# YixunLiang/UniTEX

Hardware: AMD Instinct MI355X
Metric: denoising-steps/sec (higher is better)
Workload: dtype bf16

## Files before the change

unitex_amd/_lib.py:

```python
import ctypes as C
import os

_HERE = os.path.dirname(os.path.abspath(__file__))
LIB_PATH = os.path.join(_HERE, "lib", "libunitex_hip.so")

c_void_p, c_long, c_int, c_float = C.c_void_p, C.c_long, C.c_int, C.c_float


class GemmDesc(C.Structure):
    _fields_ = [("A", c_void_p), ("lda", c_long), ("B", c_void_p), ("ldb", c_long),
                ("A2", c_void_p), ("lda2", c_long), ("B2", c_void_p), ("ldb2", c_long),
                ("M", c_int), ("N", c_int), ("K", c_int), ("K2", c_int),
                ("lora_n_limit", c_int), ("lora_seg_n", c_int), ("alpha", c_float),
                ("bias", c_void_p), ("gelu_from", c_int), ("gate", c_void_p),
                ("res", c_void_p), ("ldres", c_long), ("C", c_void_p), ("ldc", c_long),
                ("n_split", c_int), ("C1", c_void_p), ("ldc1", c_long), ("ntn", c_int),
                ("conv_Hi", c_int), ("conv_Wi", c_int), ("conv_Wo", c_int), ("conv_cin_log2", c_int),
                ("conv_stride", c_int), ("conv_pad", c_int), ("conv_up", c_int), ("zero_page", c_void_p),
                ("a_scale", c_void_p), ("lds_a", c_long), ("b_scale", c_void_p), ("lds_b", c_long), ("mx8", c_int),
                ("qk_cols", c_int), ("qk_tok_off", c_int), ("qk_eps", c_float), ("qk_q_scale", c_float),
                ("qk_wq", c_void_p), ("qk_wk", c_void_p), ("qk_cos", c_void_p), ("qk_sin", c_void_p),
                ("qk_Qh", c_void_p), ("qk_Kh", c_void_p), ("qk_hs", c_long),
                ("sk_work", c_void_p), ("sk_work_bytes", C.c_size_t),
                ("q_out", c_void_p), ("ldq_out", c_long), ("qs_out", c_void_p), ("qs_out_rb", c_long), ("q_out_kt0", c_int)]
# ... 177 lines not shown
    "utx_to_u8": (c_int, [c_void_p, c_void_p, c_long, c_long, c_int, c_void_p, c_void_p]),
}

_lib = None


def use_ablation_library():
    global LIB_PATH
    if _lib is not None:
        raise RuntimeError("the library is already loaded")
    LIB_PATH = os.path.join(_HERE, "lib", "libunitex_hip_ablate.so")


def load_library():
    global _lib
    if _lib is not None:
        return _lib
    if not os.path.exists(LIB_PATH):
        raise RuntimeError(
            "libunitex_hip.so not found at %s -- run `python unitex_amd/csrc/build.py` "
            "(or __graft_entry__.build()). There is no CPU/PyTorch fallback by design." % LIB_PATH)
    import torch
    lib = C.CDLL(LIB_PATH)
    for name, (res, args) in SYMBOLS.items():
        fn = getattr(lib, name)
        fn.restype = res
        fn.argtypes = args
    _lib = lib
    return lib


OPTION_NAMES = ["UTX_ATTN_GLDS", "UTX_ATTN_FAST", "UTX_ATTN_Q64", "UTX_ATTN_TPB", "UTX_ATTN_TAILSPLIT",
                "UTX_GEMM_GROUP_M", "UTX_GEMM_TILE", "UTX_GEMM_TAILSPLIT", "UTX_GEMM_PERS_GRID", "UTX_GEMM_PERS_SCHED",
                "UTX_GEMM_STREAMK", "UTX_BVH_STACK_WALK", "UTX_BVH_PACKET", "UTX_ATTN_PEEL", "UTX_ATTN8_PEEL", "UTX_NN_GRID", "UTX_GEMM_FASTK"]


def set_option(name, value):
    rc = load_library().utx_set_option(name.encode(), int(value))
    if rc != 0:
        raise ValueError("utx_set_option(%s) -> %d (%s)" % (name, rc, "ablation-only switch: not in this library" if rc == -7 else "unknown option"))


def get_options():
    lib, out = load_library(), {}
    for n in OPTION_NAMES:
        v = c_int()
        if lib.utx_get_option(n.encode(), C.byref(v)) == 0:
            out[n] = v.value
    return out


def check_abi():
    lib = load_library()
    n = len(ABI_STRUCTS)
    out = (c_int * n)()
    m = lib.utx_abi_sizes(out, n)
    if m != n:
        raise RuntimeError("ABI mismatch: library reports %d descriptor structs, binding has %d" % (m, n))
    for i, st in enumerate(ABI_STRUCTS):
        if C.sizeof(st) != out[i]:
            raise RuntimeError("ABI mismatch for %s: ctypes %d vs C %d" % (st.__name__, C.sizeof(st), out[i]))
    return True


class Context:

    def __init__(self, device=0):
# ... 32 lines not shown
```

unitex_amd/csrc/capi.cpp:

```cpp
#include <cstdint>
#include <hip/hip_runtime.h>
#include <stdio.h>
#include <string.h>
#include <string>
#include <stdlib.h>
#include <mutex>
#include <map>
#include <vector>
#include <utility>
#include "kernels.h"
#include "common.h"

UtxOptions g_utx_opt = {1, 2, 1, 1, 1, 0, 0, 0, 0, 0, 1, 0, 0, 0, 0, 1, 1, 1, 1, 0};

struct OptName { const char* name; int UtxOptions::*field; bool ablation; };
static const OptName kOptions[] = {
    {"UTX_ATTN_GLDS", &UtxOptions::attn_glds, false},       {"UTX_ATTN_FAST", &UtxOptions::attn_fast, false},
    {"UTX_ATTN_Q64", &UtxOptions::attn_q64, false},         {"UTX_ATTN_TPB", &UtxOptions::attn_tpb, false},
    {"UTX_ATTN_TAILSPLIT", &UtxOptions::attn_tailsplit, false},
    {"UTX_GEMM_GROUP_M", &UtxOptions::gemm_group_m, false}, {"UTX_GEMM_TILE", &UtxOptions::gemm_tile, false},
    {"UTX_GEMM_TAILSPLIT", &UtxOptions::gemm_tailsplit, false}, {"UTX_GEMM_PERS_GRID", &UtxOptions::gemm_pers_grid, false},
    {"UTX_GEMM_PERS_SCHED", &UtxOptions::gemm_pers_sched, false}, {"UTX_GEMM_STREAMK", &UtxOptions::gemm_streamk, false},
    {"UTX_BVH_STACK_WALK", &UtxOptions::bvh_stack_walk, false}, {"UTX_BVH_PACKET", &UtxOptions::bvh_packet, false},
    {"UTX_ATTN_PEEL", &UtxOptions::attn_peel, false},             {"UTX_ATTN8_PEEL", &UtxOptions::attn8_peel, false},
    {"UTX_NN_GRID", &UtxOptions::nn_grid, false},                 {"UTX_GEMM_FASTK", &UtxOptions::gemm_fastk, false},
    {"UTX_ATTN_VAR", &UtxOptions::attn_var_abl, true},      {"UTX_ATTN_DEBUG", &UtxOptions::attn_debug_abl, true},
    {"UTX_GEMM_DEBUG", &UtxOptions::gemm_debug_abl, true},
};
#ifdef UTX_ABLATION
static const bool kAblationBuild = true;
#else
static const bool kAblationBuild = false;
#endif

static void options_from_env_once() {
    static std::once_flag once;
    std::call_once(once, [] {
        for (const OptName& o : kOptions) {
            if (o.ablation && !kAblationBuild) continue;
            const char* e = getenv(o.name);
            if (e && *e) g_utx_opt.*(o.field) = atoi(e);
        }
    });
}

struct utx_ctx {
    int device;
    std::string err;
    std::mutex ws_mu;
    std::map<hipStream_t, std::pair<void*, size_t>> attn_ws;
    std::vector<void*> retired;
};

static void* ctx_attn_ws(utx_ctx* ctx, int H, int Sq, int S, hipStream_t stream, size_t* bytes) {
    *bytes = 0;
    if (!ctx) return nullptr;
    const size_t need = utx_attn_workspace_bytes_impl(H, Sq == S ? 0 : Sq, S, utx_ncu());
    if (need == 0) return nullptr;
// ... 429 lines not shown
```

unitex_amd/csrc/gemm_w4.hip:

```cpp
#include "common.h"
#include "kernels.h"
#include "gemm_w4_loop_asm.inc"

#ifndef W4_ZERO_BY_MFMA
#define W4_ZERO_BY_MFMA 1
#endif
#define W4_STAGE 65536

__device__ __forceinline__ float w4_gelu_tanh(float x) {
    const float k0 = 0.7978845608028654f, k1 = 0.044715f;
    const float u = k0 * (x + k1 * x * x * x);
    return x * __builtin_amdgcn_rcpf(1.0f + __expf(-2.0f * u));
}

__device__ __forceinline__ void w4_dma(unsigned lds_addr, unsigned voff, const char* sbase) {
    asm volatile("s_mov_b32 m0, %0\n\ts_nop 0\n\tglobal_load_lds_dwordx4 %1, %2" : : "s"(lds_addr), "v"(voff), "s"(sbase) : "memory");
}
__device__ __forceinline__ void w4_dma_m0(unsigned voff, const char* sbase) {
    asm volatile("global_load_lds_dwordx4 %0, %1" : : "v"(voff), "s"(sbase) : "memory");
}

#define W4_FENCE() __builtin_amdgcn_sched_barrier(0)

__device__ __forceinline__ const char* w4_uniform(const char* p) {
    const unsigned long v = (unsigned long)p;
    const unsigned lo = __builtin_amdgcn_readfirstlane((unsigned)v), hi = __builtin_amdgcn_readfirstlane((unsigned)(v >> 32));
    return (const char*)(((unsigned long)hi << 32) | lo);
}

template <bool GATED, bool QKF = false, bool MX = false, bool FK = false>
__global__ __launch_bounds__(256) __attribute__((amdgpu_waves_per_eu(1, 1))) void gemm256_w4_kernel(GemmParams p, int ntiles, int reserved , int sk_T, int sk_S) {
    extern __shared__ __attribute__((aligned(16))) char smem[];
    const int tid = threadIdx.x;
    const int lane = tid & 63;
    const int wave = __builtin_amdgcn_readfirstlane(tid >> 6);
    const int wm = wave >> 1, wn = wave & 1;
    const int l31 = lane & 31, lh = lane >> 5;
    const int G = gridDim.x;
    const int wid = xcd_remap(blockIdx.x, G);
    const int ntn = p.ntn & 0xffff, group_m = (p.ntn >> 16) & 0xff;
    const int ntm_ = (p.M + 255) / 256;
    const int per_group = group_m * ntn;
    const int nss1 = p.K / 64, nss2 = p.K2 / 64;
    const unsigned ldaB = (unsigned)p.lda * 2, ldbB = (unsigned)p.ldb * 2, lda2B = (unsigned)p.lda2 * 2, ldb2B = (unsigned)p.ldb2 * 2;
    const int nfull_tiles = ntiles - sk_T;
    const int nssu = nss1 + ((p.K2 > 0 && p.lora_n_limit > 0) ? nss2 : 0);
#define W4_NEXT_SEG(tj_, tile_, ok_, k0_, k1_)                                                     \
    do {                                                                                           \
        ok_ = false; k0_ = 0; k1_ = -1;                                                            \
        if (tj_ < 0) {                                                                             \
            tile_ += G;                                                                            \
            if (tile_ < nfull_tiles) ok_ = true; else tj_ = 0;                                     \
        }                                                                                          \
        if (!ok_) {                                                                                \
            const int r_ = wid + tj_ * G;                                                          \
            if (r_ < sk_T * sk_S) {                                                                \
                const int j_ = r_ / sk_T;                                                          \
                ok_ = true; tile_ = nfull_tiles + r_ - j_ * sk_T; ++tj_;                           \
                k0_ = (j_ * nssu) / sk_S; k1_ = ((j_ + 1) * nssu) / sk_S;                          \
            }                                                                                      \
        }                                                                                          \
    } while (0)

#define W4_TILE_ORIGIN(w_, m0_, n0_)                                                       \
// ... 412 lines not shown
                W4_RES_LOAD(rb0, 1, 0); W4_RES_LOAD(rb1, 1, 1); W4_RES_LOAD(rb2, 1, 2); W4_RES_LOAD(rb3, 1, 3);         \
                W4_RES_LOAD(rb4, 1, 4); W4_RES_LOAD(rb5, 1, 5); W4_RES_LOAD(rb6, 1, 6); W4_RES_LOAD(rb7, 1, 7);         \
                W4_FENCE();                                                                                            \
                W4_GATE_BLOCK(0, ra, 15, 1, true)                                                                      \
                W4_GATE_BLOCK(1, rb, 23, 1, true)                                                                      \
                W4_GATE_BLOCK(2, ra, 30, -1, false)                                                                    \
                W4_GATE_BLOCK(3, rb, 22, -1, false)                                                                    \
            } else {                                                                                                   \
                W4_GATE_SLOW_BLOCK(0) W4_GATE_SLOW_BLOCK(1) W4_GATE_SLOW_BLOCK(2) W4_GATE_SLOW_BLOCK(3)                \
            }                                                                                                          \
        } else if (QKF && c_n0 < p.qk_cols) {                                                                         \
                                             \
            const int col0 = c_n0 + wn * 128, dq = p.qk_cols >> 1;                                                      \
            const bool isk = col0 >= dq;                                                                               \
            const int head = (isk ? col0 - dq : col0) >> 7;                                                            \
            const float qs = isk ? 1.0f : p.qk_q_scale;                                                                \
            const int qsrow0 = p.qk_tok_off + c_m0 + wm * 128, qsrow_max = p.qk_tok_off + p.M - 1;                      \
            const unsigned qvo = (unsigned)((elane >> 4) * 256 + (elane & 15) * 16);                                    \
            const char* const qdst = (const char*)(isk ? p.qk_Kh : p.qk_Qh);                                          \
            const unsigned qhead = (unsigned)head * (unsigned)p.qk_hs * 2u;         \
            W4_QK_BLOCK(0) W4_QK_BLOCK(1) W4_QK_BLOCK(2) W4_QK_BLOCK(3)                                                \
        } else if (MX && !GATED && do_gelu && p.q_out) {                                                              \
                     \
            const int qc0 = c_n0 + wn * 128 - p.gelu_from;                                                             \
            uint8_t* const mxq_b = (uint8_t*)p.q_out + (long)(c_m0 + wm * 128) * p.ldq_out + qc0;                      \
            const unsigned mxq_vo = (unsigned)((elane >> 4) * (unsigned)p.ldq_out + (unsigned)(elane & 15) * 8u);      \
            uint32_t* const mxq_s = (uint32_t*)p.qs_out + ((long)(p.q_out_kt0 + (qc0 >> 7)) * p.qs_out_rb + ((c_m0 >> 7) + wm)) * 128; \
            W4_MXQ_BLOCK(0) W4_MXQ_BLOCK(1) W4_MXQ_BLOCK(2) W4_MXQ_BLOCK(3)                                            \
        } else {                                                                                                       \
            if (do_gelu) { W4_PLAIN_BLOCK(0, true) W4_PLAIN_BLOCK(1, true) W4_PLAIN_BLOCK(2, true) W4_PLAIN_BLOCK(3, true) } \
            else { W4_PLAIN_BLOCK(0, false) W4_PLAIN_BLOCK(1, false) W4_PLAIN_BLOCK(2, false) W4_PLAIN_BLOCK(3, false) } \
        }                                                                                                              \
    } while (0)

#define W4_DUMP(slot_)                                                                                                 \
    do {                                                                                                               \
        int dlane = lane;                                                                                              \
        asm volatile("" : "+v"(dlane));                                                                                \
        float* const wsb = (float*)p.sk_work + ((long)(slot_) * 4 + wave) * 16384 + dlane * 4;                         \
        _Pragma("unroll") for (int jn_ = 0; jn_ < 4; ++jn_)                                                            \
        _Pragma("unroll") for (int im_ = 0; im_ < 4; ++im_)                                                            \
        _Pragma("unroll") for (int a_ = 0; a_ < 4; ++a_) {                                                             \
            const w4_f32x4 v_ = {W4_ACC(jn_, im_, 4 * a_), W4_ACC(jn_, im_, 4 * a_ + 1), W4_ACC(jn_, im_, 4 * a_ + 2), W4_ACC(jn_, im_, 4 * a_ + 3)}; \
            *reinterpret_cast<w4_f32x4*>(wsb + ((jn_ * 4 + im_) * 4 + a_) * 256) = v_;                                 \
        }                                                                                                              \
    } while (0)

#define W4_STAGE_HALF(isb_) do { W4_DMA(isb_, 0); W4_DMA(isb_, 1); W4_DMA(isb_, 2); W4_DMA(isb_, 3); W4_DMA(isb_, 4); W4_DMA(isb_, 5); W4_DMA(isb_, 6); W4_DMA(isb_, 7); } while (0)
    W4_STAGE_AT(0, -1, false);
#define W4_XREAD16(FA_, FB_, base_, xlo_, xhi_)                                                            \
    W4_XREAD(0, FA_, FB_, base_, xlo_, xhi_); W4_XREAD(1, FA_, FB_, base_, xlo_, xhi_); W4_XREAD(2, FA_, FB_, base_, xlo_, xhi_); W4_XREAD(3, FA_, FB_, base_, xlo_, xhi_);     \
    W4_XREAD(4, FA_, FB_, base_, xlo_, xhi_); W4_XREAD(5, FA_, FB_, base_, xlo_, xhi_); W4_XREAD(6, FA_, FB_, base_, xlo_, xhi_); W4_XREAD(7, FA_, FB_, base_, xlo_, xhi_);     \
    W4_XREAD(8, FA_, FB_, base_, xlo_, xhi_); W4_XREAD(9, FA_, FB_, base_, xlo_, xhi_); W4_XREAD(10, FA_, FB_, base_, xlo_, xhi_); W4_XREAD(11, FA_, FB_, base_, xlo_, xhi_);   \
    W4_XREAD(12, FA_, FB_, base_, xlo_, xhi_); W4_XREAD(13, FA_, FB_, base_, xlo_, xhi_); W4_XREAD(14, FA_, FB_, base_, xlo_, xhi_); W4_XREAD(15, FA_, FB_, base_, xlo_, xhi_);
    if constexpr (MX) {
        W4_STAGE_HALF(0); W4_STAGE_HALF(1);
        W4_XSCALE_LOAD(sa_nxt, s_pSA); W4_XSCALE_LOAD(sb_nxt, s_pSB);
        W4_STAGE_ADVANCE();
        W4_DMA(0, 0); W4_DMA(0, 1); W4_DMA(0, 2); W4_DMA(0, 3); W4_DMA(0, 4); W4_DMA(0, 5); W4_DMA(0, 6); W4_DMA(0, 7);
        W4_DMA(1, 0); W4_DMA(1, 1); W4_DMA(1, 2);
        W4_WAIT_VM(11);
        W4_LANDED2(sa_nxt, sb_nxt);
        W4_FENCE();
        W4_XSCALE_TAKE();
        W4_COMPUTE_AT(0, -1);
        __builtin_amdgcn_s_barrier();
// ... 4 lines not shown
    } else {
    W4_STAGE_HALF(0); W4_STAGE_HALF(1); W4_STAGE_ADVANCE();
    W4_DMA(0, 0); W4_DMA(0, 1); W4_DMA(0, 2); W4_DMA(0, 3); W4_DMA(0, 4); W4_DMA(0, 5);
    asm volatile("s_waitcnt vmcnt(6)" ::: "memory");
    W4_COMPUTE_AT(0, -1);
    __builtin_amdgcn_s_barrier();
    W4_FENCE();
#pragma unroll
    for (int r = 0; r < 8; ++r) W4_READ(r, fa0, fb0, 0, xk0);
    asm volatile("s_waitcnt lgkmcnt(0)" ::: "memory");
    W4_FENCE();
    }

    unsigned w4f_ra[2][4], w4f_rb[2][4];
    if constexpr (FK && !MX) {
        const int xk_[4] = {xk0, xk1, xk2, xk3};
#pragma unroll
        for (int sl = 0; sl < 2; ++sl)
#pragma unroll
            for (int k = 0; k < 4; ++k) { w4f_ra[sl][k] = lds0 + (unsigned)(sl * W4_STAGE + arow + xk_[k]); w4f_rb[sl][k] = lds0 + (unsigned)(sl * W4_STAGE + brow + xk_[k]); }
    }
    for (;;) {
        if constexpr (FK && !MX) {
            if (c_slot == 0) {
                int n_ = (s_seg_end - s_ss - 1) >> 1;
                const int nc_ = (c_nss - c_ss - 1) >> 1;
                if (nc_ < n_) n_ = nc_;
                if (n_ > 0) {
                    const unsigned long pa_ = (unsigned long)s_pA, pb_ = (unsigned long)s_pB;
                    const unsigned w4f_pa_lo = __builtin_amdgcn_readfirstlane((unsigned)pa_), w4f_pa_hi = __builtin_amdgcn_readfirstlane((unsigned)(pa_ >> 32));
                    const unsigned w4f_pb_lo = __builtin_amdgcn_readfirstlane((unsigned)pb_), w4f_pb_hi = __builtin_amdgcn_readfirstlane((unsigned)(pb_ >> 32));
                    const unsigned w4f_trips = __builtin_amdgcn_readfirstlane((unsigned)n_);
                    const unsigned w4f_ldsdma = __builtin_amdgcn_readfirstlane(lds0 + (unsigned)wave * 1024u);
                    asm volatile(W4F_ASM_TEXT : W4F_ASM_OUTPUTS : W4F_ASM_INPUTS : W4F_ASM_CLOBBERS);
                    s_pA += 256L * n_; s_pB += 256L * n_;
                    s_ss += 2 * n_; c_ss += 2 * n_;
                }
            }
        }
        const int cb = c_slot * W4_STAGE, nb = (c_slot ^ 1) * W4_STAGE;
#define W4_PIECE_OF(ks_, i_) ((ks_) == 3 ? (((i_) % 3) == 0 ? (i_) / 3 : -1) : (ks_) == 0 ? (((i_) % 3) == 2 ? 6 + (i_) / 3 : -1) \
                              : (ks_) == 1 ? ((((i_) % 3) == 1 && (i_) < 15) ? 11 + (i_) / 3 : -1) : -1)
#define W4_KSTEP(i_, ks_, FA_, FB_, FAn_, FBn_, base_, xk_)                                                \
        {                                                                                                  \
            constexpr int pc_ = W4_PIECE_OF(ks_, i_);                                                      \
            constexpr int isb_ = pc_ >= 8 ? 1 : 0, d_ = pc_ < 0 ? 0 : (pc_ & 7);                           \
            if constexpr (pc_ >= 0) W4_MF_M0(i_, FA_, FB_, W4_DMA_LDS(isb_, d_)); else W4_MF(i_, FA_, FB_); \
            W4_FENCE();                                                                                    \
            if ((i_) < 8) W4_READ(i_, FAn_, FBn_, base_, xk_);                                             \
            if constexpr (pc_ >= 0) W4_DMA_M0(isb_, d_);                                                   \
            W4_FENCE();                                                                                    \
        }
#define W4_KSTEP16(ks_, FA_, FB_, FAn_, FBn_, base_, xk_)                                                  \
        W4_KSTEP(0, ks_, FA_, FB_, FAn_, FBn_, base_, xk_) W4_KSTEP(1, ks_, FA_, FB_, FAn_, FBn_, base_, xk_)   \
        W4_KSTEP(2, ks_, FA_, FB_, FAn_, FBn_, base_, xk_) W4_KSTEP(3, ks_, FA_, FB_, FAn_, FBn_, base_, xk_)   \
        W4_KSTEP(4, ks_, FA_, FB_, FAn_, FBn_, base_, xk_) W4_KSTEP(5, ks_, FA_, FB_, FAn_, FBn_, base_, xk_)   \
        W4_KSTEP(6, ks_, FA_, FB_, FAn_, FBn_, base_, xk_) W4_KSTEP(7, ks_, FA_, FB_, FAn_, FBn_, base_, xk_)   \
        W4_KSTEP(8, ks_, FA_, FB_, FAn_, FBn_, base_, xk_) W4_KSTEP(9, ks_, FA_, FB_, FAn_, FBn_, base_, xk_)   \
        W4_KSTEP(10, ks_, FA_, FB_, FAn_, FBn_, base_, xk_) W4_KSTEP(11, ks_, FA_, FB_, FAn_, FBn_, base_, xk_) \
        W4_KSTEP(12, ks_, FA_, FB_, FAn_, FBn_, base_, xk_) W4_KSTEP(13, ks_, FA_, FB_, FAn_, FBn_, base_, xk_) \
        W4_KSTEP(14, ks_, FA_, FB_, FAn_, FBn_, base_, xk_) W4_KSTEP(15, ks_, FA_, FB_, FAn_, FBn_, base_, xk_)
#define W4_XPIECE_OF(ks_, i_) ((ks_) == 1 ? ((((i_) % 3) != 2) ? ((i_) / 3) * 2 + ((i_) % 3) : -1) : (((((i_) % 3) != 2) && (i_) < 7) ? 11 + ((i_) / 3) * 2 + ((i_) % 3) : -1))
#define W4_XKSTEP(i_, ks_, FA_, FB_, FAn_, FBn_, base_, xlo_, xhi_)                                        \
        {                                                                                                  \
            constexpr int pc_ = W4_XPIECE_OF(ks_, i_);                                                     \
            constexpr int isb_ = pc_ >= 8 ? 1 : 0, d_ = pc_ < 0 ? 0 : (pc_ & 7);                           \
            if constexpr (pc_ >= 0) W4_XMF_M0(i_, ks_, FA_, FB_, xlds + (unsigned)(isb_ * 32768 + d_ * 4096)); else W4_XMF(i_, ks_, FA_, FB_); \
            W4_FENCE();                                                                                    \
            W4_XREAD(i_, FAn_, FBn_, base_, xlo_, xhi_);                                                   \
            if constexpr (pc_ >= 0) W4_DMA_M0(isb_, d_);                                                   \
            if constexpr ((ks_) == 0 && (i_) == 0) W4_XSCALE_LOAD(sa_nxt, s_pSA);                          \
            if constexpr ((ks_) == 0 && (i_) == 1) W4_XSCALE_LOAD(sb_nxt, s_pSB);                          \
            W4_FENCE();                                                                                    \
        }
#define W4_XKSTEP16(ks_, FA_, FB_, FAn_, FBn_, base_, xlo_, xhi_)                                          \
        W4_XKSTEP(0, ks_, FA_, FB_, FAn_, FBn_, base_, xlo_, xhi_) W4_XKSTEP(1, ks_, FA_, FB_, FAn_, FBn_, base_, xlo_, xhi_)   \
        W4_XKSTEP(2, ks_, FA_, FB_, FAn_, FBn_, base_, xlo_, xhi_) W4_XKSTEP(3, ks_, FA_, FB_, FAn_, FBn_, base_, xlo_, xhi_)   \
        W4_XKSTEP(4, ks_, FA_, FB_, FAn_, FBn_, base_, xlo_, xhi_) W4_XKSTEP(5, ks_, FA_, FB_, FAn_, FBn_, base_, xlo_, xhi_)   \
        W4_XKSTEP(6, ks_, FA_, FB_, FAn_, FBn_, base_, xlo_, xhi_) W4_XKSTEP(7, ks_, FA_, FB_, FAn_, FBn_, base_, xlo_, xhi_)   \
        W4_XKSTEP(8, ks_, FA_, FB_, FAn_, FBn_, base_, xlo_, xhi_) W4_XKSTEP(9, ks_, FA_, FB_, FAn_, FBn_, base_, xlo_, xhi_)   \
        W4_XKSTEP(10, ks_, FA_, FB_, FAn_, FBn_, base_, xlo_, xhi_) W4_XKSTEP(11, ks_, FA_, FB_, FAn_, FBn_, base_, xlo_, xhi_) \
        W4_XKSTEP(12, ks_, FA_, FB_, FAn_, FBn_, base_, xlo_, xhi_) W4_XKSTEP(13, ks_, FA_, FB_, FAn_, FBn_, base_, xlo_, xhi_) \
        W4_XKSTEP(14, ks_, FA_, FB_, FAn_, FBn_, base_, xlo_, xhi_) W4_XKSTEP(15, ks_, FA_, FB_, FAn_, FBn_, base_, xlo_, xhi_)
        if constexpr (MX) {
            unsigned xlds = lds_w + (unsigned)s_slot * W4_STAGE;
            W4_XKSTEP16(0, xa0, xb0, xa1, xb1, cb, xk2, xk3)
            W4_STAGE_ADVANCE();
            xlds = lds_w + (unsigned)s_slot * W4_STAGE;
            asm volatile("s_waitcnt lgkmcnt(0)" ::: "memory");
            W4_WAIT_VM(0);
            W4_LANDED2(sa_nxt, sb_nxt);
            W4_FENCE();
            __builtin_amdgcn_s_barrier();
            W4_FENCE();
            W4_XKSTEP16(1, xa1, xb1, xa0, xb0, nb, xk0, xk1)
            asm volatile("s_waitcnt lgkmcnt(0)" ::: "memory");
            W4_FENCE();
            W4_XSCALE_TAKE();
            W4_FENCE();
        } else {
        W4_KSTEP16(0, fa0, fb0, fa1, fb1, cb, xk1)
        asm volatile("s_waitcnt lgkmcnt(0)" ::: "memory");
        W4_FENCE();
        W4_KSTEP16(1, fa1, fb1, fa0, fb0, cb, xk2)
        W4_STAGE_ADVANCE();
        asm volatile("s_waitcnt lgkmcnt(0)" ::: "memory");
        W4_FENCE();
        W4_KSTEP16(2, fa0, fb0, fa1, fb1, cb, xk3)
        asm volatile("s_waitcnt lgkmcnt(0)" ::: "memory");
        asm volatile("s_waitcnt vmcnt(0)" ::: "memory");
        W4_FENCE();
        __builtin_amdgcn_s_barrier();
        W4_FENCE();
        W4_KSTEP16(3, fa1, fb1, fa0, fb0, nb, xk0)
        asm volatile("s_waitcnt lgkmcnt(0)" ::: "memory");
        W4_FENCE();
        }
        c_slot ^= 1;
        ++c_ss;
        if (c_ss != c_nss) continue;
        const bool full = (c_m0 + 256 <= p.M);
        W4_MFMA_DRAIN();
        if (c_tj > 0) { W4_DUMP(wid + (c_tj - 1) * G); }
        else W4_EPILOGUE();
        W4_ZERO_ACC()
        if constexpr (MX) {
            const int rb = c_slot * W4_STAGE;
            W4_XREAD16(xa0, xb0, rb, xk0, xk1)
            asm volatile("s_waitcnt lgkmcnt(0)" ::: "memory");
            W4_FENCE();
        }
        if constexpr (QKF) {
            const int rb = c_slot * W4_STAGE;
#pragma unroll
            for (int r = 0; r < 8; ++r) W4_READ(r, fa0, fb0, rb, xk0);
            asm volatile("s_waitcnt lgkmcnt(0)" ::: "memory");
            W4_FENCE();
        }
        bool done;
        W4_COMPUTE_NEXT(done);
        if (done) break;
    }
    asm volatile("s_waitcnt vmcnt(0)" ::: "memory");
}

template <bool GATED>
__global__ __launch_bounds__(256) void gemm_w4_fixup_kernel(GemmParams p, int ntiles, int sk_T, int sk_S) {
    typedef __attribute__((ext_vector_type(4))) float f32x4v;
    const int t = blockIdx.x >> 4, wv = (blockIdx.x >> 2) & 3, im = blockIdx.x & 3;
    const int tid = threadIdx.x, lane = tid & 63, jn = tid >> 6, l31 = lane & 31, lh = lane >> 5;
    const int wm = wv >> 1, wn = wv & 1;
    const int ntn = p.ntn & 0xffff, group_m = (p.ntn >> 16) & 0xff, ntm = (p.M + 255) / 256, per_group = group_m * ntn;
    const int w = ntiles - sk_T + t;
    const int grp = w / per_group, rem = w - grp * per_group, ftm = grp * group_m;
    const int gs = (ntm - ftm < group_m) ? ntm - ftm : group_m;
    const int tn = rem / gs;
    const int m0 = (ftm + rem - tn * gs) * 256, n0 = tn * 256;
    f32x4v acc[4];
#pragma unroll
    for (int a = 0; a < 4; ++a) acc[a] = f32x4v{0.f, 0.f, 0.f, 0.f};
    for (int j = 0; j < sk_S; ++j) {
        const float* src = (const float*)p.sk_work + ((long)(j * sk_T + t) * 4 + wv) * 16384 + (jn * 4 + im) * 1024 + lane * 4;
#pragma unroll
        for (int a = 0; a < 4; ++a) acc[a] += *reinterpret_cast<const f32x4v*>(src + a * 256);
    }
    const int m = m0 + wm * 128 + im * 32 + l31;
    if (m >= p.M) return;
    const bool do_gelu = !GATED && n0 >= p.gelu_from, to_c1 = !GATED && n0 >= p.n_split;
    bf16_t* const crow = to_c1 ? (bf16_t*)p.C1 + (long)m * p.ldc1 - p.n_split : (bf16_t*)p.C + (long)m * p.ldc;
#pragma unroll
    for (int a = 0; a < 4; ++a) {
        const int n = n0 + wn * 128 + jn * 32 + 8 * a + 4 * lh;
        float v[4];
// ... 39 lines not shown
    const int nssu = p.K / 64 + ((p.K2 > 0 && p.lora_n_limit > 0) ? p.K2 / 64 : 0);
    if (opt >= 1000) {
        const int S = opt - 1000;
        if (S >= 2 && S <= 8 && nssu >= S && T * S <= 2 * grid) { *T_out = T; *S_out = S; }
        return;
    }
    const int margin = opt > 1 ? opt : 4;
    int best = nssu - margin, bestS = 0;
    for (int S = 2; S <= 8; ++S) {
        if (nssu / S < 8 || T * S > 2 * grid) break;
        const int passes = (T * S + grid - 1) / grid;
        const int est = passes * ((nssu + S - 1) / S + 4) + 6 + (8 * T * S) / 256;
        if (est < best) { best = est; bestS = S; }
    }
    if (bestS) { *T_out = T; *S_out = bestS; }
}

extern "C" int utx_launch_gemm_w4(GemmParams p, hipStream_t stream) {
    constexpr int LDS = 2 * W4_STAGE + 4 * 8192;
    UTX_ONCE_PER_DEVICE(attr_set) {
        const void* ks[2] = {reinterpret_cast<const void*>(gemm256_w4_kernel<false>), reinterpret_cast<const void*>(gemm256_w4_kernel<true>)};
        for (const void* k : ks)
            if (hipFuncSetAttribute(k, hipFuncAttributeMaxDynamicSharedMemorySize, LDS) != hipSuccess) return -3;
        UTX_ONCE_DONE(attr_set);
    }
    const int ncu = utx_ncu();
    const int ntm = (p.M + 255) / 256, ntn = p.N / 256;
    int group_m = g_utx_opt.gemm_group_m > 0 ? g_utx_opt.gemm_group_m : (ntn >= 32 ? 8 : 2);
    if (group_m > ntm) group_m = ntm;
    p.ntn = ntn | (group_m << 16);
    const int tiles = ntm * ntn;
    int grid = tiles < ncu ? tiles : ncu;
    if (g_utx_opt.gemm_pers_grid > 0 && g_utx_opt.gemm_pers_grid < grid) grid = g_utx_opt.gemm_pers_grid;
    int sk_T = 0, sk_S = 0;
    utx_gemm_w4_split_plan(&p, tiles, grid, (p.sk_work && p.sk_work_bytes >= (size_t)2 * grid * 262144) ? 1 : 0, &sk_T, &sk_S);
    if (p.mx8 == 2) {
        if (p.K2 > 0 || p.qk_cols > 0 || (p.K % 64) || !p.a_scale || !p.b_scale || p.lds_a < (p.M + 127) / 128 || p.lds_b < p.N / 128 ||
            ((uintptr_t)p.a_scale & 15) || ((uintptr_t)p.b_scale & 15)) return -2;
        if (p.gate && (p.gelu_from < p.N || p.n_split < p.N)) return -2;
        if (p.q_out && (p.gate || !p.qs_out || p.gelu_from >= p.N || (p.gelu_from % 128) || (p.ldq_out & 7) || p.ldq_out < p.N - p.gelu_from ||
                        p.qs_out_rb < (p.M + 127) / 128 || p.q_out_kt0 < 0 || ((uintptr_t)p.qs_out & 15) || ((uintptr_t)p.q_out & 7))) return -2;
        UTX_ONCE_PER_DEVICE(ax) {
            if (hipFuncSetAttribute(reinterpret_cast<const void*>(gemm256_w4_kernel<false, false, true>), hipFuncAttributeMaxDynamicSharedMemorySize, LDS) != hipSuccess ||
                hipFuncSetAttribute(reinterpret_cast<const void*>(gemm256_w4_kernel<true, false, true>), hipFuncAttributeMaxDynamicSharedMemorySize, LDS) != hipSuccess) return -3;
            UTX_ONCE_DONE(ax);
        }
        if (p.gate) hipLaunchKernelGGL((gemm256_w4_kernel<true, false, true>), dim3(grid), dim3(256), LDS, stream, p, tiles, 0, sk_T, sk_S);
        else hipLaunchKernelGGL((gemm256_w4_kernel<false, false, true>), dim3(grid), dim3(256), LDS, stream, p, tiles, 0, sk_T, sk_S);
    } else if (g_utx_opt.gemm_fastk != 0) {
        UTX_ONCE_PER_DEVICE(af) {
            const void* kf[3] = {reinterpret_cast<const void*>(gemm256_w4_kernel<false, false, false, true>), reinterpret_cast<const void*>(gemm256_w4_kernel<true, false, false, true>),
                                 reinterpret_cast<const void*>(gemm256_w4_kernel<false, true, false, true>)};
            for (const void* k : kf)
                if (hipFuncSetAttribute(k, hipFuncAttributeMaxDynamicSharedMemorySize, LDS) != hipSuccess) return -3;
            UTX_ONCE_DONE(af);
        }
        if (p.gate) {
            if (p.gelu_from < p.N || p.n_split < p.N) return -2;
            hipLaunchKernelGGL((gemm256_w4_kernel<true, false, false, true>), dim3(grid), dim3(256), LDS, stream, p, tiles, 0, sk_T, sk_S);
        } else if (p.qk_cols > 0) hipLaunchKernelGGL((gemm256_w4_kernel<false, true, false, true>), dim3(grid), dim3(256), LDS, stream, p, tiles, 0, sk_T, sk_S);
        else hipLaunchKernelGGL((gemm256_w4_kernel<false, false, false, true>), dim3(grid), dim3(256), LDS, stream, p, tiles, 0, sk_T, sk_S);
    } else if (p.gate) {
        if (p.gelu_from < p.N || p.n_split < p.N) return -2;
        hipLaunchKernelGGL((gemm256_w4_kernel<true>), dim3(grid), dim3(256), LDS, stream, p, tiles, 0, sk_T, sk_S);
    } else {
        if (p.qk_cols > 0) {
            UTX_ONCE_PER_DEVICE(aq) { if (hipFuncSetAttribute(reinterpret_cast<const void*>(gemm256_w4_kernel<false, true>), hipFuncAttributeMaxDynamicSharedMemorySize, LDS) != hipSuccess) return -3; UTX_ONCE_DONE(aq); }
            hipLaunchKernelGGL((gemm256_w4_kernel<false, true>), dim3(grid), dim3(256), LDS, stream, p, tiles, 0, sk_T, sk_S);
        } else
        hipLaunchKernelGGL((gemm256_w4_kernel<false>), dim3(grid), dim3(256), LDS, stream, p, tiles, 0, sk_T, sk_S);
    }
    if (sk_T > 0) {
        if (p.gate) hipLaunchKernelGGL((gemm_w4_fixup_kernel<true>), dim3(sk_T * 16), dim3(256), 0, stream, p, tiles, sk_T, sk_S);
        else hipLaunchKernelGGL((gemm_w4_fixup_kernel<false>), dim3(sk_T * 16), dim3(256), 0, stream, p, tiles, sk_T, sk_S);
    }
    return hipGetLastError() == hipSuccess ? 0 : -4;
}
```

unitex_amd/csrc/kernels.h:

```cpp
#pragma once
#include <hip/hip_runtime.h>
#include <stdint.h>
#include "../../include/unitex_hip.h"
#ifndef UTX_BF16_T
#define UTX_BF16_T
typedef uint16_t bf16_t;
#endif

struct AttnParams {
    const bf16_t* q;
    const bf16_t* k;
    const bf16_t* vt;
    bf16_t* o;
    long q_hs, q_ss, k_hs, k_ss, vt_hs, vt_ds, o_ss;
    int H, S, nqb;
    int Sq;
    int dbg;
    float scale_log2;
    unsigned char* flags;
    int flag_hs;
    int w_base, nsplit, tiles_per_split;
    bf16_t* part_o;
    float* part_lse;
    float key_bias_log2;
// ... 7 lines not shown
    const uint8_t *q8, *k8;
    const uint8_t* v8t;
    const uint32_t *qs, *ks;
    const uint32_t* vs;
    bf16_t* o;
    long o_ss;
    int H, S, Sq, S_pad, nqb;
    float key_bias_log2;
    int key_bias_period;
    int w_base, nsplit, tiles_per_split;
    bf16_t* part_o;
    float* part_lse;
    void* work;
    size_t work_bytes;
};
struct UtxOptions {
    int attn_glds;
    int attn_fast;
    int attn_q64;
    int attn_tpb;
    int attn_tailsplit;
    int gemm_group_m;
    int gemm_tile;
    int gemm_tailsplit;
    int gemm_pers_grid;
    int gemm_pers_sched;
    int gemm_streamk;
    int bvh_stack_walk;
    int attn_var_abl, attn_debug_abl, gemm_debug_abl;
    int bvh_packet;
    int attn_peel;
    int attn8_peel;
    int gemm_fastk;
    int nn_grid;
};
extern UtxOptions g_utx_opt;

typedef utx_gemm_desc GemmParams;
typedef utx_knn_desc KnnParams;
typedef utx_gemv_desc GemvParams;
typedef utx_qkv_post_desc QkvPostParams;
typedef utx_ln_mod_desc LnModParams;
typedef utx_sched_desc SchedParams;

extern "C" {
int utx_launch_attn_fwd(const void* q, const void* k, const void* vt, void* o,
                        long q_hs, long q_ss, long k_hs, long k_ss, long vt_hs, long vt_ds,
                        long o_ss, int H, int S, int Sq, float scale, float key_bias_log2, int key_bias_period, void* work, size_t work_bytes, hipStream_t stream);
void utx_attn_split_plan_impl(int H, int Sq, int S, int ncu, int out[4]);
size_t utx_attn_workspace_bytes_impl(int H, int Sq, int S, int ncu);
size_t utx_attn_split_bytes_impl(int H, int Sq, int S, int ncu);
size_t utx_attn_q64_flag_bytes(int H, int Sq, int S);
int utx_attn_q64_takes(const AttnParams* p, int presc);
int utx_launch_attn_merge(const AttnParams* t, int n_items, hipStream_t stream);
int utx_launch_attn_fwd_glds(const AttnParams* p, int presc, hipStream_t stream);
int utx_launch_attn_fwd_fp8(const Attn8Params* p, hipStream_t stream);
int utx_launch_quant_vt_mx8(const void* vt, void* v8, void* vs, int H, int S_pad, hipStream_t stream);
int utx_launch_attn_fwd_blk(const void* q, const void* k, const void* vt, void* o, long q_hs, long q_ss, long k_hs, long k_ss, long vt_hs, long vt_ds,
                            long o_ss, int H, int S, int Sq, float scale, float key_bias_log2, int key_bias_period, void* work, size_t work_bytes,
                            int blk_rows, long q_bs, long k_bs, long vt_bs, hipStream_t stream);
int utx_launch_attn_fwd_q64(const AttnParams* p, int presc, hipStream_t stream);
int utx_launch_gemm_bf16(const GemmParams* p, hipStream_t stream);
size_t utx_gemm_streamk_workspace_bytes_impl(void);
void utx_gemm_plan_impl(const GemmParams* p, int ncu, int sk_has_work, int out[4]);
void utx_gemm_w4_split_plan(const GemmParams* p, int tiles, int grid, int has_work, int* T, int* S);
int utx_launch_gemm_w4(GemmParams p, hipStream_t stream);
// ... 48 lines not shown
```

Measured before the change: 0.5705.

## Park GEMM epilogue outputs in registers and drain stores during next tile's K-loop

Adds a 'park' epilogue path to the persistent W4 GEMM kernel for non-gated, non-QK, non-MX variants. Accumulators for the last three row-blocks are scaled, biased, GELU'd and packed to bf16 in registers instead of being written immediately. Their LDS staging and nontemporal global stores are then interleaved into the first K-tiles of the next output tile through per-kstep hooks. If there is no next tile, or the next tile is short, they are flushed directly. This aims to hide epilogue store latency behind MFMA work, at the cost of many extra live VGPRs and more complex scheduling. It is enabled by default through a new UTX_GEMM_PARK option.

Result: slower. 0.5499 (-3.6%).

```diff
diff --git a/unitex_amd/_lib.py b/unitex_amd/_lib.py
--- a/unitex_amd/_lib.py
+++ b/unitex_amd/_lib.py
@@ -233,7 +233,7 @@
 
 OPTION_NAMES = ["UTX_ATTN_GLDS", "UTX_ATTN_FAST", "UTX_ATTN_Q64", "UTX_ATTN_TPB", "UTX_ATTN_TAILSPLIT",
                 "UTX_GEMM_GROUP_M", "UTX_GEMM_TILE", "UTX_GEMM_TAILSPLIT", "UTX_GEMM_PERS_GRID", "UTX_GEMM_PERS_SCHED",
-                "UTX_GEMM_STREAMK", "UTX_BVH_STACK_WALK", "UTX_BVH_PACKET", "UTX_ATTN_PEEL", "UTX_ATTN8_PEEL", "UTX_NN_GRID", "UTX_GEMM_FASTK"]
+                "UTX_GEMM_STREAMK", "UTX_BVH_STACK_WALK", "UTX_BVH_PACKET", "UTX_ATTN_PEEL", "UTX_ATTN8_PEEL", "UTX_NN_GRID", "UTX_GEMM_FASTK", "UTX_GEMM_PARK"]
 
 
 def set_option(name, value):
diff --git a/unitex_amd/csrc/capi.cpp b/unitex_amd/csrc/capi.cpp
--- a/unitex_amd/csrc/capi.cpp
+++ b/unitex_amd/csrc/capi.cpp
@@ -11,7 +11,7 @@
 #include "kernels.h"
 #include "common.h"
 
-UtxOptions g_utx_opt = {1, 2, 1, 1, 1, 0, 0, 0, 0, 0, 1, 0, 0, 0, 0, 1, 1, 1, 1, 0};
+UtxOptions g_utx_opt = {1, 2, 1, 1, 1, 0, 0, 0, 0, 0, 1, 0, 0, 0, 0, 1, 1, 1, 1, 1, 0};
 
 struct OptName { const char* name; int UtxOptions::*field; bool ablation; };
 static const OptName kOptions[] = {
@@ -24,6 +24,7 @@
     {"UTX_BVH_STACK_WALK", &UtxOptions::bvh_stack_walk, false}, {"UTX_BVH_PACKET", &UtxOptions::bvh_packet, false},
     {"UTX_ATTN_PEEL", &UtxOptions::attn_peel, false},             {"UTX_ATTN8_PEEL", &UtxOptions::attn8_peel, false},
     {"UTX_NN_GRID", &UtxOptions::nn_grid, false},                 {"UTX_GEMM_FASTK", &UtxOptions::gemm_fastk, false},
+    {"UTX_GEMM_PARK", &UtxOptions::gemm_park, false},
     {"UTX_ATTN_VAR", &UtxOptions::attn_var_abl, true},      {"UTX_ATTN_DEBUG", &UtxOptions::attn_debug_abl, true},
     {"UTX_GEMM_DEBUG", &UtxOptions::gemm_debug_abl, true},
 };
diff --git a/unitex_amd/csrc/gemm_w4.hip b/unitex_amd/csrc/gemm_w4.hip
--- a/unitex_amd/csrc/gemm_w4.hip
+++ b/unitex_amd/csrc/gemm_w4.hip
@@ -29,7 +29,7 @@
 }
 
 template <bool GATED, bool QKF = false, bool MX = false, bool FK = false>
-__global__ __launch_bounds__(256) __attribute__((amdgpu_waves_per_eu(1, 1))) void gemm256_w4_kernel(GemmParams p, int ntiles, int reserved , int sk_T, int sk_S) {
+__global__ __launch_bounds__(256) __attribute__((amdgpu_waves_per_eu(1, 1))) void gemm256_w4_kernel(GemmParams p, int ntiles, int park , int sk_T, int sk_S) {
     extern __shared__ __attribute__((aligned(16))) char smem[];
     const int tid = threadIdx.x;
     const int lane = tid & 63;
@@ -508,6 +508,97 @@
             else { W4_PLAIN_BLOCK(0, false) W4_PLAIN_BLOCK(1, false) W4_PLAIN_BLOCK(2, false) W4_PLAIN_BLOCK(3, false) } \
         }                                                                                                              \
     } while (0)
+
+#ifndef W4_PARK_FIRST
+#define W4_PARK_FIRST 1
+#endif
+    constexpr bool PARKABLE = !GATED && !QKF && !MX;
+#define W4_PARK_BLOCK(im_, GELU_)                                                                                      \
+        _Pragma("unroll") for (int jn_ = 0; jn_ < 4; ++jn_)                                                            \
+            _Pragma("unroll") for (int q_ = 0; q_ < 2; ++q_) {                                                         \
+                float b8_[8];                                                                                          \
+                _Pragma("unroll") for (int h_ = 0; h_ < 2; ++h_)                                                       \
+                    _Pragma("unroll") for (int d_ = 0; d_ < 2; ++d_) {                                                 \
+                        const uint32_t w_ = bsel[jn_][q_][2 * h_ + d_];                                                \
+                        b8_[4 * h_ + 2 * d_] = p.bias ? bf2f((uint16_t)(w_ & 0xffff)) : 0.f;                           \
+                        b8_[4 * h_ + 2 * d_ + 1] = p.bias ? bf2f((uint16_t)(w_ >> 16)) : 0.f;                          \
+                    }                                                                                                  \
+                float v_[8];                                                                                           \
+                _Pragma("unroll") for (int c_ = 0; c_ < 8; ++c_) {                                                     \
+                    v_[c_] = W4_ACC(jn_, im_, 8 * q_ + c_) * p.alpha + b8_[c_];                                        \
+                    if (GELU_) v_[c_] = w4_gelu_tanh(rbf(v_[c_]));                                                     \
+                }                                                                                                      \
+                pk[im_][jn_][q_][0] = pack2bf(v_[0], v_[1]); pk[im_][jn_][q_][1] = pack2bf(v_[2], v_[3]);              \
+                pk[im_][jn_][q_][2] = pack2bf(v_[4], v_[5]); pk[im_][jn_][q_][3] = pack2bf(v_[6], v_[7]);              \
+                W4_FENCE();       \
+            }
+#define W4_PARK_TILE()                                                                                                 \
+    do {                                                                                                               \
+        int el31 = l31, elh = lh, elane = lane;                                                                        \
+        asm volatile("" : "+v"(el31), "+v"(elh), "+v"(elane));                                                         \
+        const uint32_t hm = 0u - (uint32_t)elh;                                                                        \
+        const bool do_gelu = c_n0 >= p.gelu_from;                                                                      \
+        const bool to_c1 = c_n0 >= p.n_split;                                                                          \
+        bf16_t* const cbase = to_c1 ? (bf16_t*)p.C1 : (bf16_t*)p.C;                                                    \
+        pk_ldc = to_c1 ? p.ldc1 : p.ldc;                                                                               \
+        pk_wofs = el31 * 256; pk_wxor = ((el31 & 15) ^ elh) << 4;                                                      \
+        pk_rofs = (elane >> 4) * 256 + (((elane & 15) ^ (elane >> 4)) << 4);                                           \
+        pk_rowg = c_m0 + wm * 128 + (elane >> 4);                                                                      \
+        pk_rows = p.M - (c_m0 + wm * 128);              \
+        pk_cub = (char*)cbase + ((long)(c_m0 + wm * 128) * pk_ldc + (c_n0 + wn * 128 - (to_c1 ? p.n_split : 0))) * 2;  \
+        pk_cvo = (unsigned)((elane >> 4) * (unsigned)pk_ldc * 2u + (unsigned)(elane & 15) * 16u);                      \
+        const int wofs = pk_wofs, wxor = pk_wxor;                                                                      \
+        const bf16_t* const ebias = (const bf16_t*)(p.bias ? p.bias : p.B) + c_n0 + wn * 128;                          \
+        w4_u32x16 bq0, bq1, bq2, bq3;                                                                                  \
+        uint32_t bsel[4][2][4];                                                                                        \
+        W4_SLOAD64(bq0, bq1, bq2, bq3, ebias);                                                                         \
+        _Pragma("unroll") for (int jn_ = 0; jn_ < 4; ++jn_) {                                                          \
+            const w4_u32x16 bw_ = jn_ == 0 ? bq0 : jn_ == 1 ? bq1 : jn_ == 2 ? bq2 : bq3;                              \
+            _Pragma("unroll") for (int q_ = 0; q_ < 2; ++q_)                                                           \
+                _Pragma("unroll") for (int e_ = 0; e_ < 4; ++e_)                                                       \
+                    bsel[jn_][q_][e_] = (bw_[8 * q_ + 4 * (e_ >> 1) + 2 + (e_ & 1)] & hm) | (bw_[8 * q_ + 4 * (e_ >> 1) + (e_ & 1)] & ~hm); \
+        }                                                                                                              \
+        const long ldc = pk_ldc; char* const cub = pk_cub; const unsigned cvo = pk_cvo; const int rofs = pk_rofs, rowg = pk_rowg;       \
+        if (do_gelu) { W4_PARK_BLOCKS(true) } else { W4_PARK_BLOCKS(false) }                                           \
+    } while (0)
+#define W4_PARK_ONE(im_, GELU_)                                                                                        \
+        if constexpr ((im_) < W4_PARK_FIRST) { W4_PLAIN_BLOCK(im_, GELU_) }                                            \
+        else if constexpr ((im_) == W4_PARK_FIRST) { W4_EPI_WRITE(im_, GELU_) }                                        \
+        else { W4_PARK_BLOCK(im_, GELU_) }
+#define W4_PARK_BLOCKS(GELU_) W4_PARK_ONE(0, GELU_) W4_PARK_ONE(1, GELU_) W4_PARK_ONE(2, GELU_) W4_PARK_ONE(3, GELU_)
+#define W4_PK_STAGE(im_, jn_, q_)                                                                                      \
+        {                                                                                                              \
+            auto s0_ = __builtin_amdgcn_permlane32_swap(pk[im_][jn_][q_][0], pk[im_][jn_][q_][2], false, false);       \
+            auto s1_ = __builtin_amdgcn_permlane32_swap(pk[im_][jn_][q_][1], pk[im_][jn_][q_][3], false, false);       \
+            *reinterpret_cast<uint4*>(stg + pk_wofs + (((4 * (jn_) + 2 * (q_)) << 4) ^ pk_wxor)) = make_uint4(s0_[0], s1_[0], s0_[1], s1_[1]); \
+        }
+#define W4_PK_READ(t_) pky[t_] = *reinterpret_cast<const uint4*>(stg + (t_) * 1024 + (pk_rofs ^ (64 * ((t_) & 3))));
+#define W4_PK_STORE(im_, t_)                                                                                           \
+        if (32 * (im_) + 32 <= pk_rows || pk_rowg + 32 * (im_) + 4 * (t_) < p.M) {                                     \
+            const w4_u32x4 ov_ = {pky[t_].x, pky[t_].y, pky[t_].z, pky[t_].w};                                         \
+            __builtin_nontemporal_store(ov_, reinterpret_cast<w4_u32x4*>(pk_cub + (long)(32 * (im_) + 4 * (t_)) * pk_ldc * 2 + pk_cvo)); \
+        }
+#define W4_DRAIN_SLOT(d_, ks_, i_)                                                                                     \
+        {                                                                                                              \
+            constexpr int s_ = 16 * (ks_) + (i_);                                                                      \
+            if constexpr (s_ >= 4 && s_ <= 18 && (s_ & 1) == 0) { W4_PK_STORE(d_, ((s_ - 4) >> 1) & 7) }               \
+            if constexpr (s_ <= 14 && (s_ & 1) == 0) { W4_PK_READ((s_ >> 1) & 7) }                                     \
+            if constexpr ((d_) < 3 && (ks_) == 2 && (i_) < 8) W4_PK_STAGE(((d_) + 1) & 3, ((i_) & 7) >> 1, (i_) & 1)   \
+        }
+#define W4_DRAIN0(ks_, i_) W4_DRAIN_SLOT(W4_PARK_FIRST, ks_, i_)
+#define W4_DRAIN1(ks_, i_) W4_DRAIN_SLOT(W4_PARK_FIRST + 1, ks_, i_)
+#define W4_DRAIN2(ks_, i_) W4_DRAIN_SLOT(W4_PARK_FIRST + 2, ks_, i_)
+#define W4_DRAIN3(ks_, i_) W4_DRAIN_SLOT(W4_PARK_FIRST + 3, ks_, i_)
+#define W4_PK_FLUSH(im_, staged_)                                                                                      \
+        {                                                                                                              \
+            if (!(staged_)) {                                                                                          \
+                W4_PK_STAGE(im_, 0, 0) W4_PK_STAGE(im_, 0, 1) W4_PK_STAGE(im_, 1, 0) W4_PK_STAGE(im_, 1, 1)            \
+                W4_PK_STAGE(im_, 2, 0) W4_PK_STAGE(im_, 2, 1) W4_PK_STAGE(im_, 3, 0) W4_PK_STAGE(im_, 3, 1)            \
+            }                                                                                                          \
+            W4_PK_READ(0) W4_PK_READ(1) W4_PK_READ(2) W4_PK_READ(3) W4_PK_READ(4) W4_PK_READ(5) W4_PK_READ(6) W4_PK_READ(7) \
+            W4_PK_STORE(im_, 0) W4_PK_STORE(im_, 1) W4_PK_STORE(im_, 2) W4_PK_STORE(im_, 3)                            \
+            W4_PK_STORE(im_, 4) W4_PK_STORE(im_, 5) W4_PK_STORE(im_, 6) W4_PK_STORE(im_, 7)                            \
+        }
 
 #define W4_DUMP(slot_)                                                                                                 \
     do {                                                                                                               \
@@ -578,6 +669,13 @@
                     const unsigned w4f_pb_lo = __builtin_amdgcn_readfirstlane((unsigned)pb_), w4f_pb_hi = __builtin_amdgcn_readfirstlane((unsigned)(pb_ >> 32));
                     const unsigned w4f_trips = __builtin_amdgcn_readfirstlane((unsigned)n_);
                     const unsigned w4f_ldsdma = __builtin_amdgcn_readfirstlane(lds0 + (unsigned)wave * 1024u);
+                    if constexpr (PARKABLE) {
+                        int ar_ = arow, br_ = brow;
+                        asm volatile("" : "+v"(ar_), "+v"(br_));
+                        const int xk_[4] = {xk0, xk1, xk2, xk3};
+                        _Pragma("unroll") for (int sl = 0; sl < 2; ++sl)
+                            _Pragma("unroll") for (int k = 0; k < 4; ++k) { w4f_ra[sl][k] = lds0 + (unsigned)(sl * W4_STAGE + ar_ + xk_[k]); w4f_rb[sl][k] = lds0 + (unsigned)(sl * W4_STAGE + br_ + xk_[k]); }
+                    }
                     asm volatile(W4F_ASM_TEXT : W4F_ASM_OUTPUTS : W4F_ASM_INPUTS : W4F_ASM_CLOBBERS);
                     s_pA += 256L * n_; s_pB += 256L * n_;
                     s_ss += 2 * n_; c_ss += 2 * n_;
@@ -587,7 +685,7 @@
         const int cb = c_slot * W4_STAGE, nb = (c_slot ^ 1) * W4_STAGE;
 #define W4_PIECE_OF(ks_, i_) ((ks_) == 3 ? (((i_) % 3) == 0 ? (i_) / 3 : -1) : (ks_) == 0 ? (((i_) % 3) == 2 ? 6 + (i_) / 3 : -1) \
                               : (ks_) == 1 ? ((((i_) % 3) == 1 && (i_) < 15) ? 11 + (i_) / 3 : -1) : -1)
-#define W4_KSTEP(i_, ks_, FA_, FB_, FAn_, FBn_, base_, xk_)                                                \
+#define W4_KSTEP(i_, ks_, FA_, FB_, FAn_, FBn_, base_, xk_, HOOK_)                                         \
         {                                                                                                  \
             constexpr int pc_ = W4_PIECE_OF(ks_, i_);                                                      \
             constexpr int isb_ = pc_ >= 8 ? 1 : 0, d_ = pc_ < 0 ? 0 : (pc_ & 7);                           \
@@ -595,17 +693,40 @@
             W4_FENCE();                                                                                    \
             if ((i_) < 8) W4_READ(i_, FAn_, FBn_, base_, xk_);                                             \
             if constexpr (pc_ >= 0) W4_DMA_M0(isb_, d_);                                                   \
+            HOOK_(ks_, i_)                                                                                 \
             W4_FENCE();                                                                                    \
         }
-#define W4_KSTEP16(ks_, FA_, FB_, FAn_, FBn_, base_, xk_)                                                  \
-        W4_KSTEP(0, ks_, FA_, FB_, FAn_, FBn_, base_, xk_) W4_KSTEP(1, ks_, FA_, FB_, FAn_, FBn_, base_, xk_)   \
-        W4_KSTEP(2, ks_, FA_, FB_, FAn_, FBn_, base_, xk_) W4_KSTEP(3, ks_, FA_, FB_, FAn_, FBn_, base_, xk_)   \
-        W4_KSTEP(4, ks_, FA_, FB_, FAn_, FBn_, base_, xk_) W4_KSTEP(5, ks_, FA_, FB_, FAn_, FBn_, base_, xk_)   \
-        W4_KSTEP(6, ks_, FA_, FB_, FAn_, FBn_, base_, xk_) W4_KSTEP(7, ks_, FA_, FB_, FAn_, FBn_, base_, xk_)   \
-        W4_KSTEP(8, ks_, FA_, FB_, FAn_, FBn_, base_, xk_) W4_KSTEP(9, ks_, FA_, FB_, FAn_, FBn_, base_, xk_)   \
-        W4_KSTEP(10, ks_, FA_, FB_, FAn_, FBn_, base_, xk_) W4_KSTEP(11, ks_, FA_, FB_, FAn_, FBn_, base_, xk_) \
-        W4_KSTEP(12, ks_, FA_, FB_, FAn_, FBn_, base_, xk_) W4_KSTEP(13, ks_, FA_, FB_, FAn_, FBn_, base_, xk_) \
-        W4_KSTEP(14, ks_, FA_, FB_, FAn_, FBn_, base_, xk_) W4_KSTEP(15, ks_, FA_, FB_, FAn_, FBn_, base_, xk_)
+#define W4_KSTEP16(ks_, FA_, FB_, FAn_, FBn_, base_, xk_, H_)                                              \
+        W4_KSTEP(0, ks_, FA_, FB_, FAn_, FBn_, base_, xk_, H_) W4_KSTEP(1, ks_, FA_, FB_, FAn_, FBn_, base_, xk_, H_)   \
+        W4_KSTEP(2, ks_, FA_, FB_, FAn_, FBn_, base_, xk_, H_) W4_KSTEP(3, ks_, FA_, FB_, FAn_, FBn_, base_, xk_, H_)   \
+        W4_KSTEP(4, ks_, FA_, FB_, FAn_, FBn_, base_, xk_, H_) W4_KSTEP(5, ks_, FA_, FB_, FAn_, FBn_, base_, xk_, H_)   \
+        W4_KSTEP(6, ks_, FA_, FB_, FAn_, FBn_, base_, xk_, H_) W4_KSTEP(7, ks_, FA_, FB_, FAn_, FBn_, base_, xk_, H_)   \
+        W4_KSTEP(8, ks_, FA_, FB_, FAn_, FBn_, base_, xk_, H_) W4_KSTEP(9, ks_, FA_, FB_, FAn_, FBn_, base_, xk_, H_)   \
+        W4_KSTEP(10, ks_, FA_, FB_, FAn_, FBn_, base_, xk_, H_) W4_KSTEP(11, ks_, FA_, FB_, FAn_, FBn_, base_, xk_, H_) \
+        W4_KSTEP(12, ks_, FA_, FB_, FAn_, FBn_, base_, xk_, H_) W4_KSTEP(13, ks_, FA_, FB_, FAn_, FBn_, base_, xk_, H_) \
+        W4_KSTEP(14, ks_, FA_, FB_, FAn_, FBn_, base_, xk_, H_) W4_KSTEP(15, ks_, FA_, FB_, FAn_, FBn_, base_, xk_, H_)
+#define W4_NODRAIN(ks_, i_)
+#define W4_KTILE(H_)                                                                                       \
+                                                                                        \
+        W4_KSTEP16(0, fa0, fb0, fa1, fb1, cb, xk1, H_)                                                     \
+        asm volatile("s_waitcnt lgkmcnt(0)" ::: "memory");                                                 \
+        W4_FENCE();                                                                                        \
+                                                                                        \
+        W4_KSTEP16(1, fa1, fb1, fa0, fb0, cb, xk2, H_)                                                     \
+        W4_STAGE_ADVANCE();                                                                                \
+        asm volatile("s_waitcnt lgkmcnt(0)" ::: "memory");                                                 \
+        W4_FENCE();                                                                                        \
+                                                                                        \
+        W4_KSTEP16(2, fa0, fb0, fa1, fb1, cb, xk3, H_)                                                     \
+        asm volatile("s_waitcnt lgkmcnt(0)" ::: "memory");                                                 \
+        asm volatile("s_waitcnt vmcnt(0)" ::: "memory");       \
+        W4_FENCE();                                                                                        \
+        __builtin_amdgcn_s_barrier();                                                                      \
+        W4_FENCE();                                                                                        \
+                                                                                        \
+        W4_KSTEP16(3, fa1, fb1, fa0, fb0, nb, xk0, H_)                                                     \
+        asm volatile("s_waitcnt lgkmcnt(0)" ::: "memory");                                                 \
+        W4_FENCE();
 #define W4_XPIECE_OF(ks_, i_) ((ks_) == 1 ? ((((i_) % 3) != 2) ? ((i_) / 3) * 2 + ((i_) % 3) : -1) : (((((i_) % 3) != 2) && (i_) < 7) ? 11 + ((i_) / 3) * 2 + ((i_) % 3) : -1))
 #define W4_XKSTEP(i_, ks_, FA_, FB_, FAn_, FBn_, base_, xlo_, xhi_)                                        \
         {                                                                                                  \
@@ -645,29 +766,24 @@
             W4_XSCALE_TAKE();
             W4_FENCE();
         } else {
-        W4_KSTEP16(0, fa0, fb0, fa1, fb1, cb, xk1)
-        asm volatile("s_waitcnt lgkmcnt(0)" ::: "memory");
-        W4_FENCE();
-        W4_KSTEP16(1, fa1, fb1, fa0, fb0, cb, xk2)
-        W4_STAGE_ADVANCE();
-        asm volatile("s_waitcnt lgkmcnt(0)" ::: "memory");
-        W4_FENCE();
-        W4_KSTEP16(2, fa0, fb0, fa1, fb1, cb, xk3)
-        asm volatile("s_waitcnt lgkmcnt(0)" ::: "memory");
-        asm volatile("s_waitcnt vmcnt(0)" ::: "memory");
-        W4_FENCE();
-        __builtin_amdgcn_s_barrier();
-        W4_FENCE();
-        W4_KSTEP16(3, fa1, fb1, fa0, fb0, nb, xk0)
-        asm volatile("s_waitcnt lgkmcnt(0)" ::: "memory");
-        W4_FENCE();
+        W4_KTILE(W4_NODRAIN)
         }
         c_slot ^= 1;
         ++c_ss;
         if (c_ss != c_nss) continue;
         const bool full = (c_m0 + 256 <= p.M);
         W4_MFMA_DRAIN();
+        uint32_t pk[4][4][2][4];
+        uint4 pky[8];
+        int pk_wofs = 0, pk_wxor = 0, pk_rofs = 0, pk_rowg = 0, pk_rows = 0;
+        unsigned pk_cvo = 0;
+        long pk_ldc = 0;
+        char* pk_cub = nullptr;
+        bool parked = false;
         if (c_tj > 0) { W4_DUMP(wid + (c_tj - 1) * G); }
+        else if (PARKABLE && park != 0) {
+            if constexpr (PARKABLE) { W4_PARK_TILE(); parked = true; }
+        }
         else W4_EPILOGUE();
         W4_ZERO_ACC()
         if constexpr (MX) {
@@ -676,6 +792,15 @@
             asm volatile("s_waitcnt lgkmcnt(0)" ::: "memory");
             W4_FENCE();
         }
+        if constexpr (PARKABLE) {
+            if (parked) {
+                const int rb = c_slot * W4_STAGE;
+#pragma unroll
+                for (int r = 0; r < 8; ++r) W4_READ(r, fa0, fb0, rb, xk0);
+                asm volatile("s_waitcnt lgkmcnt(0)" ::: "memory");
+                W4_FENCE();
+            }
+        }
         if constexpr (QKF) {
             const int rb = c_slot * W4_STAGE;
 #pragma unroll
@@ -685,6 +810,22 @@
         }
         bool done;
         W4_COMPUTE_NEXT(done);
+        if constexpr (PARKABLE) {
+            if (parked) {
+#define W4_DRAIN_KTILE(H_) { const int cb = c_slot * W4_STAGE, nb = (c_slot ^ 1) * W4_STAGE; W4_KTILE(H_) c_slot ^= 1; ++c_ss; }
+                if (!done && c_nss >= 5) {
+                    W4_DRAIN_KTILE(W4_DRAIN0)
+                    if constexpr (W4_PARK_FIRST < 3) W4_DRAIN_KTILE(W4_DRAIN1)
+                    if constexpr (W4_PARK_FIRST < 2) W4_DRAIN_KTILE(W4_DRAIN2)
+                    if constexpr (W4_PARK_FIRST < 1) W4_DRAIN_KTILE(W4_DRAIN3)
+                } else {
+                    if constexpr (W4_PARK_FIRST <= 0) W4_PK_FLUSH(0, W4_PARK_FIRST == 0)
+                    if constexpr (W4_PARK_FIRST <= 1) W4_PK_FLUSH(1, W4_PARK_FIRST == 1)
+                    if constexpr (W4_PARK_FIRST <= 2) W4_PK_FLUSH(2, W4_PARK_FIRST == 2)
+                    W4_PK_FLUSH(3, W4_PARK_FIRST == 3)
+                }
+            }
+        }
         if (done) break;
     }
     asm volatile("s_waitcnt vmcnt(0)" ::: "memory");
@@ -790,6 +931,7 @@
     const int tiles = ntm * ntn;
     int grid = tiles < ncu ? tiles : ncu;
     if (g_utx_opt.gemm_pers_grid > 0 && g_utx_opt.gemm_pers_grid < grid) grid = g_utx_opt.gemm_pers_grid;
+    const int park = g_utx_opt.gemm_park != 0 ? 1 : 0;
     int sk_T = 0, sk_S = 0;
     utx_gemm_w4_split_plan(&p, tiles, grid, (p.sk_work && p.sk_work_bytes >= (size_t)2 * grid * 262144) ? 1 : 0, &sk_T, &sk_S);
     if (p.mx8 == 2) {
@@ -803,8 +945,8 @@
                 hipFuncSetAttribute(reinterpret_cast<const void*>(gemm256_w4_kernel<true, false, true>), hipFuncAttributeMaxDynamicSharedMemorySize, LDS) != hipSuccess) return -3;
             UTX_ONCE_DONE(ax);
         }
-        if (p.gate) hipLaunchKernelGGL((gemm256_w4_kernel<true, false, true>), dim3(grid), dim3(256), LDS, stream, p, tiles, 0, sk_T, sk_S);
-        else hipLaunchKernelGGL((gemm256_w4_kernel<false, false, true>), dim3(grid), dim3(256), LDS, stream, p, tiles, 0, sk_T, sk_S);
+        if (p.gate) hipLaunchKernelGGL((gemm256_w4_kernel<true, false, true>), dim3(grid), dim3(256), LDS, stream, p, tiles, park, sk_T, sk_S);
+        else hipLaunchKernelGGL((gemm256_w4_kernel<false, false, true>), dim3(grid), dim3(256), LDS, stream, p, tiles, park, sk_T, sk_S);
     } else if (g_utx_opt.gemm_fastk != 0) {
         UTX_ONCE_PER_DEVICE(af) {
             const void* kf[3] = {reinterpret_cast<const void*>(gemm256_w4_kernel<false, false, false, true>), reinterpret_cast<const void*>(gemm256_w4_kernel<true, false, false, true>),
@@ -815,18 +957,18 @@
         }
         if (p.gate) {
             if (p.gelu_from < p.N || p.n_split < p.N) return -2;
-            hipLaunchKernelGGL((gemm256_w4_kernel<true, false, false, true>), dim3(grid), dim3(256), LDS, stream, p, tiles, 0, sk_T, sk_S);
-        } else if (p.qk_cols > 0) hipLaunchKernelGGL((gemm256_w4_kernel<false, true, false, true>), dim3(grid), dim3(256), LDS, stream, p, tiles, 0, sk_T, sk_S);
-        else hipLaunchKernelGGL((gemm256_w4_kernel<false, false, false, true>), dim3(grid), dim3(256), LDS, stream, p, tiles, 0, sk_T, sk_S);
+            hipLaunchKernelGGL((gemm256_w4_kernel<true, false, false, true>), dim3(grid), dim3(256), LDS, stream, p, tiles, park, sk_T, sk_S);
+        } else if (p.qk_cols > 0) hipLaunchKernelGGL((gemm256_w4_kernel<false, true, false, true>), dim3(grid), dim3(256), LDS, stream, p, tiles, park, sk_T, sk_S);
+        else hipLaunchKernelGGL((gemm256_w4_kernel<false, false, false, true>), dim3(grid), dim3(256), LDS, stream, p, tiles, park, sk_T, sk_S);
     } else if (p.gate) {
         if (p.gelu_from < p.N || p.n_split < p.N) return -2;
-        hipLaunchKernelGGL((gemm256_w4_kernel<true>), dim3(grid), dim3(256), LDS, stream, p, tiles, 0, sk_T, sk_S);
+        hipLaunchKernelGGL((gemm256_w4_kernel<true>), dim3(grid), dim3(256), LDS, stream, p, tiles, park, sk_T, sk_S);
     } else {
         if (p.qk_cols > 0) {
             UTX_ONCE_PER_DEVICE(aq) { if (hipFuncSetAttribute(reinterpret_cast<const void*>(gemm256_w4_kernel<false, true>), hipFuncAttributeMaxDynamicSharedMemorySize, LDS) != hipSuccess) return -3; UTX_ONCE_DONE(aq); }
-            hipLaunchKernelGGL((gemm256_w4_kernel<false, true>), dim3(grid), dim3(256), LDS, stream, p, tiles, 0, sk_T, sk_S);
+            hipLaunchKernelGGL((gemm256_w4_kernel<false, true>), dim3(grid), dim3(256), LDS, stream, p, tiles, park, sk_T, sk_S);
         } else
-        hipLaunchKernelGGL((gemm256_w4_kernel<false>), dim3(grid), dim3(256), LDS, stream, p, tiles, 0, sk_T, sk_S);
+        hipLaunchKernelGGL((gemm256_w4_kernel<false>), dim3(grid), dim3(256), LDS, stream, p, tiles, park, sk_T, sk_S);
     }
     if (sk_T > 0) {
         if (p.gate) hipLaunchKernelGGL((gemm_w4_fixup_kernel<true>), dim3(sk_T * 16), dim3(256), 0, stream, p, tiles, sk_T, sk_S);
diff --git a/unitex_amd/csrc/kernels.h b/unitex_amd/csrc/kernels.h
--- a/unitex_amd/csrc/kernels.h
+++ b/unitex_amd/csrc/kernels.h
@@ -63,6 +63,7 @@
     int attn_peel;
     int attn8_peel;
     int gemm_fastk;
+    int gemm_park;
     int nn_grid;
 };
 extern UtxOptions g_utx_opt;
```
